# compbio-UofT/shrimp

Measured on AMD Instinct MI355X. Metric: reads/sec mapped (whole node), 100bp LS reads vs 3Gbp ref, 1/2/4/8 GPUs, higher is better.
Workload: dtype int16

## Files before the change

shrimp_amd/csrc/gm_lookup5.hip:

```cpp
#include <algorithm>
#include <cmath>
#include <mutex>
#include "gm_common.h"
#include "gm_internal.h"
#include <rocprim/device/device_scan.hpp>

typedef uint32_t k5_u32x4 __attribute__((ext_vector_type(4), aligned(4)));
typedef __attribute__((address_space(3))) uint32_t k5_lds_u32;
#define K5_LDS(off) ((k5_lds_u32*)(uintptr_t)(uint32_t)(off))
typedef __attribute__((address_space(3))) uint16_t k5_lds_u16;
#define K5_LDS16(off) ((k5_lds_u16*)(uintptr_t)(uint32_t)(off))
#define K5_LDS_OR(off, m) __hip_atomic_fetch_or(K5_LDS(off), (m), __ATOMIC_RELAXED, __HIP_MEMORY_SCOPE_WORKGROUP)

#ifndef K5_Q
#define K5_Q 4
#endif
enum { C_NCAND = 0, C_OVERFLOW, C_NMEMB, C_NKEEP, C_NSTRIP, C_NEDGE, C_NLISTS , C_SINK = 8, C_NRAW = 9, C_NDEFER = 10, C_NCAND0 = 11 , C_SPILL = 12 , C_WORDS = 16 };
#define K5_MAX_ROUNDS 4

#ifdef K5_STAMPS
__device__ unsigned long long k5_stamps[16];
#define K5_STAMP(i) do { if (tid == 0) { const unsigned long long t_ = __builtin_amdgcn_s_memtime(); atomicAdd(&k5_stamps[i], t_ - t_prev); t_prev = t_; } } while (0)
extern "C" int gm_debug_k5_stamps(unsigned long long* out) {
  unsigned long long z[16] = {0, 0, 0, 0, 0, 0, 0, 0, 0, 0, 0, 0, 0, 0, 0, 0};
  if (hipMemcpyFromSymbol(out, HIP_SYMBOL(k5_stamps), sizeof z) != hipSuccess) return GM_E_NODEVICE;
  if (hipMemcpyToSymbol(HIP_SYMBOL(k5_stamps), z, sizeof z) != hipSuccess) return GM_E_NODEVICE;
  return GM_OK;
}
#else
#define K5_STAMP(i) do { } while (0)
#endif

#ifdef GM_TUNING
__device__ unsigned long long k5_paths[3];
extern "C" int gm_debug_k5_paths(unsigned long long* out) {
  unsigned long long z[3] = {0, 0, 0};
  if (hipMemcpyFromSymbol(out, HIP_SYMBOL(k5_paths), sizeof z) != hipSuccess) return GM_E_NODEVICE;
  if (hipMemcpyToSymbol(HIP_SYMBOL(k5_paths), z, sizeof z) != hipSuccess) return GM_E_NODEVICE;
  return GM_OK;
}
#endif

struct K5Args {
  const uint32_t* reads; int n_reads, read_len, read_words, max_n_kmers, NL;
  int lsw, ltw;
  int cand_cap, hbits;
  int cand_limit;
  int xrec;
  int rounds; uint32_t round_regs;
  uint2* spill; int spill_cap;
  uint64_t* out; uint32_t* out_cnt; int out_cap; uint32_t* surv_cnt;
  int prune; uint32_t D; int e_max;
  uint32_t* heavy_list; uint32_t* heavy_cnt; int heavy_cap;
  unsigned long long* stats;
  uint32_t* fb_list; uint32_t* fb_cnt; int fb_cap;
  uint32_t* start_flags; uint32_t start_epoch;
  uint64_t* raw_out; int raw_cap; uint32_t* surv_seg; int n_slabs; uint32_t* pl_list; uint32_t* pl_cnt; int pl_cap;
};

__device__ __forceinline__ uint32_t k5_lane_times(int lane, uint32_t W) {
  uint32_t r; asm("v_mul_u32_u24 %0, %1, %2" : "=v"(r) : "v"(lane), "s"(W)); return r;
}

#include "gm_region_table.h"

#define K5_KERNEL_HEAD template <int LSWC> __global__ void __launch_bounds__(1024) k_lookup_v5(GmIndexDev ix, K5Args a)
#define K5_KERNEL_MULTI false
#include "gm_lookup5_kernel.inc"
#undef K5_KERNEL_HEAD
#undef K5_KERNEL_MULTI
#define K5_KERNEL_HEAD __global__ void __launch_bounds__(1024) __attribute__((amdgpu_waves_per_eu(5, 5))) k_lookup_v5_rounds(GmIndexDev ix, K5Args a)
#define K5_KERNEL_MULTI true
#define K5_KERNEL_LSWC 15
#include "gm_lookup5_kernel.inc"
#undef K5_KERNEL_HEAD
#undef K5_KERNEL_MULTI
#undef K5_KERNEL_LSWC
#define K5_KERNEL_HEAD __global__ void __launch_bounds__(1024) __attribute__((amdgpu_waves_per_eu(5, 5))) k_lookup_v5_half(GmIndexDev ix, K5Args a)
#define K5_KERNEL_MULTI true
#define K5_KERNEL_LSWC 14
#define K5_KERNEL_BLOOM true
#include "gm_lookup5_kernel.inc"
#undef K5_KERNEL_HEAD
#undef K5_KERNEL_BLOOM
#ifdef GM_TUNING
#define K5_KERNEL_HEAD __global__ void __launch_bounds__(1024) __attribute__((amdgpu_waves_per_eu(5, 5))) k_lookup_v5_half_plain(GmIndexDev ix, K5Args a)
#define K5_KERNEL_BLOOM false
#include "gm_lookup5_kernel.inc"
#undef K5_KERNEL_HEAD
#undef K5_KERNEL_BLOOM
#endif
#undef K5_KERNEL_MULTI
#undef K5_KERNEL_LSWC

__device__ __forceinline__ bool k5_strip(uint32_t p, int rb, uint32_t ovl) { return (p & ((1u << rb) - 1u)) < ovl && (p >> rb) > 0u; }

__global__ void __launch_bounds__(256) k_strip_count(const uint32_t* __restrict__ pos, uint32_t n_pos, int rb, uint32_t ovl, uint32_t* __restrict__ grp_cnt, uint32_t n_groups) {
  const uint32_t lane = threadIdx.x & 63u;
  uint64_t g = ((uint64_t)blockIdx.x * blockDim.x + threadIdx.x) >> 6;
  const uint64_t stride = ((uint64_t)gridDim.x * blockDim.x) >> 6;
  for (; g < n_groups; g += stride) {
    const uint64_t i = g * 64 + lane;
    const bool f = i < n_pos && k5_strip(pos[i], rb, ovl);
    const unsigned long long b = __ballot(f);
    if (lane == 0) grp_cnt[g] = (uint32_t)__popcll(b);
  }
}
__global__ void __launch_bounds__(256) k_strip_scatter(const uint32_t* __restrict__ pos, uint32_t n_pos, int rb, uint32_t ovl, const uint32_t* __restrict__ grp_rank,
                                                       uint32_t n_groups, uint32_t* __restrict__ spos) {
  const uint32_t lane = threadIdx.x & 63u;
  uint64_t g = ((uint64_t)blockIdx.x * blockDim.x + threadIdx.x) >> 6;
  const uint64_t stride = ((uint64_t)gridDim.x * blockDim.x) >> 6;
  for (; g < n_groups; g += stride) {
    const uint64_t i = g * 64 + lane;
    const uint32_t p = i < n_pos ? pos[i] : 0u;
    const bool f = i < n_pos && k5_strip(p, rb, ovl);
    const unsigned long long b = __ballot(f);
    if (f) spos[grp_rank[g] + (uint32_t)__popcll(b & ((1ull << lane) - 1ull))] = p;
  }
}
__global__ void __launch_bounds__(256) k_strip_dir(const uint32_t* __restrict__ dir, const uint32_t* __restrict__ pos, uint32_t n_pos, uint64_t K, int S, int rb, uint32_t ovl,
                                                   const uint32_t* __restrict__ grp_rank, uint32_t* __restrict__ sdir) {
  uint64_t k = (uint64_t)blockIdx.x * blockDim.x + threadIdx.x;
  const uint64_t stride = (uint64_t)gridDim.x * blockDim.x;
  for (; k <= K; k += stride) {
    const uint32_t i = dir[k * (uint64_t)S];
    uint32_t r = grp_rank[i >> 6];
    for (uint32_t q = i & ~63u; q < i; q++) r += k5_strip(pos[q], rb, ovl) ? 1u : 0u;
    sdir[k] = r;
  }
}

static std::mutex g_strip_mutex;
int gm_index_derive_strips(GmIndexHost* ix, hipStream_t stream) {
  std::lock_guard<std::mutex> lock(g_strip_mutex);
  if (ix->strips_ready) return GM_OK;
  const int rb = ix->params.region_bits; const uint32_t ovl = (uint32_t)ix->params.region_overlap;
  for (int sn = 0; sn < ix->n_seeds; sn++) {
    GmSeedHost& sd = ix->seeds[sn];
    const uint64_t K = 1ull << sd.kbits;
    const uint32_t n_groups = (uint32_t)(((uint64_t)sd.n_pos + 63) / 64) + 1u;
    uint32_t *d_cnt = nullptr, *d_rank = nullptr; void* tmp = nullptr; size_t tmp_bytes = 0;
    GM_HIP(hipMalloc(&d_cnt, (size_t)n_groups * 4)); GM_HIP(hipMalloc(&d_rank, (size_t)n_groups * 4));
    hipLaunchKernelGGL(k_strip_count, dim3(256 * 16), dim3(256), 0, stream, sd.d_pos, sd.n_pos, rb, ovl, d_cnt, n_groups);
    hipError_t e = rocprim::exclusive_scan(nullptr, tmp_bytes, d_cnt, d_rank, 0u, (size_t)n_groups, rocprim::plus<uint32_t>(), stream);
    if (e != hipSuccess) { gm_set_error("exclusive_scan size query: %s", hipGetErrorString(e)); return GM_E_NODEVICE; }
    GM_HIP(hipMalloc(&tmp, tmp_bytes ? tmp_bytes : 16));
    e = rocprim::exclusive_scan(tmp, tmp_bytes, d_cnt, d_rank, 0u, (size_t)n_groups, rocprim::plus<uint32_t>(), stream);
    if (e != hipSuccess) { gm_set_error("exclusive_scan: %s", hipGetErrorString(e)); return GM_E_NODEVICE; }
    uint32_t total = 0;
    GM_HIP(hipMemcpyAsync(&total, d_rank + (n_groups - 1), 4, hipMemcpyDeviceToHost, stream));
    GM_HIP(hipStreamSynchronize(stream));
    sd.n_spos = total;
    GM_HIP(hipMalloc(&sd.d_spos, ((size_t)total + 64) * 4));
    GM_HIP(hipMemsetAsync(sd.d_spos, 0xff, ((size_t)total + 64) * 4, stream));
    GM_HIP(hipMalloc(&sd.d_sdir, (size_t)(K + 1 + 16) * 4));
    hipLaunchKernelGGL(k_strip_scatter, dim3(256 * 16), dim3(256), 0, stream, sd.d_pos, sd.n_pos, rb, ovl, d_rank, n_groups, sd.d_spos);
    hipLaunchKernelGGL(k_strip_dir, dim3(256 * 16), dim3(256), 0, stream, sd.d_dir, sd.d_pos, sd.n_pos, K, ix->n_slabs, rb, ovl, d_rank, sd.d_sdir);
    GM_HIP(hipGetLastError());
    GM_HIP(hipStreamSynchronize(stream));
    (void)hipFree(d_cnt); (void)hipFree(d_rank); (void)hipFree(tmp);
  }
  ix->strips_ready = true;
  return GM_OK;
}

int gm_lookup5_launch(const GmIndexDev& ix, const uint32_t* d_reads, int n_reads, int read_len, int read_words, int max_n_kmers, int NL,
                      uint64_t* d_out, uint32_t* d_out_cnt, int out_cap, uint32_t* d_surv_cnt, int prune, uint32_t D, int e_max,
                      uint32_t* d_heavy_list, uint32_t* d_heavy_cnt, int heavy_cap, unsigned long long* d_stats, hipStream_t stream, GmK1Scratch* K,
                      uint64_t* d_raw, int raw_cap, uint32_t* d_surv_seg) {
  int dev = 0; if (hipGetDevice(&dev) != hipSuccess) return 0;
  if (!ix.seed[0].sdir || ix.region_bits < 9 || ix.region_bits > 16 || NL <= 0) return 0;
  const bool forced = gm_tune("GM_K1_V5") != nullptr;
  double entries = 0;
  for (int sn = 0; sn < ix.n_seeds; sn++) {
    const double lists = std::max(0, read_len - ix.seed[sn].span + 1 - ix.colour);
    entries += lists * (double)ix.seed[sn].n_pos / (double)(1ull << (ix.hflag ? 2 * GM_HASH_TABLE_POWER : 2 * ix.seed[sn].weight));
  }
  if (!forced && entries < 8000.0) return 0;
  const size_t budget = 160 * 1024 - 512;
  const size_t fixed0 = (size_t)24 * NL + 2 * (size_t)((read_len + 15) & ~15) + C_WORDS * 4 + GM_MAX_SEEDS * 32;
  const size_t full_tables = (size_t)(4u << 15) + (size_t)(4u << 12);
  int xrec = read_len > 128 ? 16 : 64;
  if (fixed0 + 24 * (size_t)xrec + full_tables > budget && fixed0 + 24 * 16 + full_tables <= budget) xrec = (int)((budget - full_tables - fixed0) / 24);
  const size_t fixed = fixed0 + 24 * (size_t)xrec;
  int lsw = 15;
  int threads = 1024;
  bool small_shape = false;
  if (!forced && ix.colour && NL <= 512 && !gm_tune("GM_K5_LSW") && !gm_tune("GM_K1_THREADS") && !(gm_tune("GM_K5_SMALL") && atoi(gm_tune("GM_K5_SMALL")) == 0)) {
    const double lam = entries * (double)((1u << ix.region_bits) + ix.region_overlap) / std::max(1.0, (double)ix.total_len);
    const double memb = 2.0 * entries * std::min(1.0, lam), late = 0.5 * entries * std::min(1.0, entries / (double)(32ull << 14));
    const double first = entries * std::min(1.0, (late + 0.5 * memb) / (double)(32ull << 11));
    const double cap14 = (double)(((4u << 14) / 4u / 6u) & ~15u);
    if (memb + late + first <= 0.5 * cap14 && fixed + (size_t)(4u << 14) + (size_t)(4u << 11) <= 96 * 1024) { small_shape = true; lsw = 14; threads = 512; }
  }
  int half = 0;
  if (const char* e = gm_tune("GM_K5_HALF")) half = atoi(e);
  const size_t half_budget = 80 * 1024 - 512, half_tables = (size_t)(4u << 14) + (size_t)(4u << 11);
  if (half && (ix.region_bits < 11 || NL > 512 || fixed0 + 24 * 8 + half_tables > half_budget)) half = 0;
  if (half) { lsw = 14; threads = 512; xrec = (int)std::min<size_t>(64, (half_budget - half_tables - fixed0) / 24); }
  if (half) if (const char* e = gm_tune("GM_K5_HALF_THREADS")) threads = std::max(64, std::min(1024, atoi(e) & ~63));
  const size_t fixed_h = fixed0 + 24 * (size_t)xrec;
  if (!half)
  if (const char* e = gm_tune("GM_K5_LSW")) lsw = std::max(8, std::min(15, atoi(e)));
  while (!half && lsw >= 8 && fixed + (size_t)(4u << lsw) + (size_t)(4u << (lsw - 3)) > budget) lsw--;
  if (lsw < 8) return 0;
  if (!half)
  if (const char* e = gm_tune("GM_K1_THREADS")) { const int v = std::max(64, std::min(1024, atoi(e))); threads = 64; while (threads * 2 <= v) threads *= 2; }
  const int ltw = lsw - 3;
  const int hbits = lsw - 2;
  const int cand_cap = (int)(((4u << lsw) / 4u / 6u) & ~15u);
  if (cand_cap < 16) return 0;
  int cand_limit = cand_cap - 8, rounds = 1;
  if (!forced) {
    const double lam = entries * (double)((1u << ix.region_bits) + ix.region_overlap) / std::max(1.0, (double)ix.total_len);
    const double memb = 2.0 * entries * std::min(1.0, lam), late = 0.5 * entries * std::min(1.0, entries / (double)(32ull << (lsw + (half == 1 ? 1 : 0))));
    const double first = entries * std::min(1.0, (late + 0.5 * memb) / (double)(32ull << (lsw - 3)));
    if (memb + late + first > 0.85 * cand_cap) {
      rounds = (int)std::ceil((memb + late + first) / ((half ? 0.95 : 1.25) * cand_cap));
      rounds = std::max(rounds, 2);
      if (rounds > K5_MAX_ROUNDS || NL > threads || lsw != (half ? 14 : 15)) return 0;
    }
  }
  if (const char* e = gm_tune("GM_K5_ROUNDS")) { rounds = std::max(1, std::min(K5_MAX_ROUNDS, atoi(e))); if (rounds > 1 && (NL > threads || lsw != (half ? 14 : 15))) return 0; }
  const uint32_t n_regs = (uint32_t)((ix.total_len + (1ull << ix.region_bits) - 1) >> ix.region_bits);
  const uint32_t round_regs = std::max(1u, (n_regs + (uint32_t)rounds - 1u) / (uint32_t)rounds);
  if (const char* e = gm_tune("GM_K5_CANDLIMIT")) cand_limit = std::max(1, std::min(cand_limit, atoi(e)));
  if (prune && (D + (uint32_t)std::max(0, e_max) > (1u << ix.region_bits) || D > 0xFFFFu)) return 0;
  const size_t lds = (half ? fixed_h : fixed) + (size_t)(4u << lsw) + (size_t)(4u << ltw);
  const int fb_cap = std::max(4096, 2 * n_reads);
  if (!K->cus) { if (hipDeviceGetAttribute(&K->cus, hipDeviceAttributeMultiprocessorCount, dev) != hipSuccess || K->cus < 1) K->cus = 256; }
  if (fb_cap > K->k5_cap) {
    if (K->k5_fb) { (void)hipStreamSynchronize(stream); (void)hipFree(K->k5_fb); (void)hipFree(K->k5_pl); K->k5_fb = nullptr; K->k5_pl = nullptr; K->k5_cap = 0; }
    if (hipMalloc(&K->k5_fb, (size_t)(fb_cap + 4) * 4) != hipSuccess) return 0;
    if (hipMalloc(&K->k5_pl, (size_t)(fb_cap + 4) * 4) != hipSuccess) return 0;
    K->k5_cap = fb_cap;
  }
  uint32_t* const fb_cnt_p = K->k5_fb + K->k5_cap; uint32_t* const pl_cnt_p = K->k5_pl + K->k5_cap;
  if (hipMemsetAsync(fb_cnt_p, 0, 4, stream) != hipSuccess || hipMemsetAsync(pl_cnt_p, 0, 4, stream) != hipSuccess) return GM_E_NODEVICE;
  if (gm_lds_at_least((const void*)k_lookup_v5<15>, lds) != hipSuccess || gm_lds_at_least((const void*)k_lookup_v5<14>, lds) != hipSuccess ||
      gm_lds_at_least((const void*)k_lookup_v5_rounds, lds) != hipSuccess || gm_lds_at_least((const void*)k_lookup_v5_half, lds) != hipSuccess ||
#ifdef GM_TUNING
      gm_lds_at_least((const void*)k_lookup_v5_half_plain, lds) != hipSuccess ||
#endif
      gm_lds_at_least((const void*)k_lookup_v5<0>, lds) != hipSuccess) return 0;
  int grid = std::min(2 * n_reads, (half || small_shape) ? 2 * K->cus : K->cus);
  if (const char* e = gm_tune("GM_K5_GRID")) grid = std::max(1, std::min(2 * n_reads, atoi(e)));
  K5Args a;
  a.reads = d_reads; a.n_reads = n_reads; a.read_len = read_len; a.read_words = read_words; a.max_n_kmers = max_n_kmers; a.NL = NL;
  a.lsw = lsw; a.ltw = ltw; a.cand_cap = cand_cap; a.hbits = hbits; a.cand_limit = cand_limit; a.xrec = xrec; a.rounds = rounds; a.round_regs = round_regs;
  a.out = d_out; a.out_cnt = d_out_cnt; a.out_cap = out_cap; a.surv_cnt = d_surv_cnt; a.prune = prune; a.D = D; a.e_max = e_max;
  a.heavy_list = d_heavy_list; a.heavy_cnt = d_heavy_cnt; a.heavy_cap = heavy_cap; a.stats = d_stats;
  a.fb_list = K->k5_fb; a.fb_cnt = fb_cnt_p; a.fb_cap = fb_cap;
  a.raw_out = prune ? d_raw : nullptr; a.raw_cap = raw_cap; a.surv_seg = d_surv_seg; a.n_slabs = ix.n_slabs; a.pl_list = K->k5_pl; a.pl_cnt = pl_cnt_p; a.pl_cap = fb_cap;
  a.spill = nullptr; a.spill_cap = cand_cap;
  if (rounds > 1) {
    const size_t need = (size_t)grid * (size_t)(rounds - 1) * (size_t)cand_cap;
    if (need > K->k5_spill_n) {
      if (K->k5_spill) { (void)hipStreamSynchronize(stream); (void)hipFree(K->k5_spill); K->k5_spill = nullptr; K->k5_spill_n = 0; }
      if (hipMalloc(&K->k5_spill, need * sizeof(uint2)) != hipSuccess) return 0;
      K->k5_spill_n = need;
    }
    a.spill = K->k5_spill;
  }
  const bool use_flags = K->start_flags && grid <= K->flag_cap;
  K->flag_grid = use_flags ? grid : 0;
  a.start_flags = use_flags ? K->start_flags : nullptr; a.start_epoch = K->epoch;
  K->rounds = rounds; K->half = half;
  if (half) {
#ifdef GM_TUNING
    if (half == 2) hipLaunchKernelGGL(k_lookup_v5_half_plain, dim3(grid), dim3(threads), lds, stream, ix, a); else
#endif
    hipLaunchKernelGGL(k_lookup_v5_half, dim3(grid), dim3(threads), lds, stream, ix, a);
  } else if (rounds > 1) hipLaunchKernelGGL(k_lookup_v5_rounds, dim3(grid), dim3(threads), lds, stream, ix, a);
  else if (lsw == 15) hipLaunchKernelGGL((k_lookup_v5<15>), dim3(grid), dim3(threads), lds, stream, ix, a);
  else if (lsw == 14) hipLaunchKernelGGL((k_lookup_v5<14>), dim3(grid), dim3(threads), lds, stream, ix, a);
  else hipLaunchKernelGGL((k_lookup_v5<0>), dim3(grid), dim3(threads), lds, stream, ix, a);
  if (hipGetLastError() != hipSuccess) return GM_E_NODEVICE;
  return 1;
}
```

shrimp_amd/csrc/gm_lookup5_kernel.inc:

```
K5_KERNEL_HEAD {
  constexpr bool MULTI = K5_KERNEL_MULTI;
#ifdef K5_KERNEL_BLOOM
  constexpr bool BLOOM = K5_KERNEL_BLOOM;
#else
  constexpr bool BLOOM = false;
#endif
#ifdef K5_KERNEL_LSWC
  constexpr int LSWC = K5_KERNEL_LSWC;
#endif
  if (a.start_flags && threadIdx.x == 0) __hip_atomic_store(&a.start_flags[blockIdx.x], a.start_epoch, __ATOMIC_RELAXED, __HIP_MEMORY_SCOPE_SYSTEM);
  __builtin_amdgcn_s_setprio(3);
  extern __shared__ __align__(16) uint32_t smem[];
  const int tid = threadIdx.x, nthr = blockDim.x, lane = tid & (GM_WAVE - 1);
  const int wv = __builtin_amdgcn_readfirstlane(tid >> 6), nwv = nthr >> 6;
  const int S = ix.n_slabs, rb = ix.region_bits, lsw = LSWC ? LSWC : a.lsw, ltw = lsw - 3, hbits = lsw - 2;
  const int cand_cap = LSWC ? (int)(((4u << LSWC) / 4u / 6u) & ~15u) : a.cand_cap;
  const uint32_t rmask = (1u << rb) - 1u, ovl = (uint32_t)ix.region_overlap;
  const uint32_t wmask = (1u << lsw) - 1u, tmask = (1u << ltw) - 1u;
  if ((uint32_t)(uintptr_t)(k5_lds_u32*)smem != 0u) __builtin_trap();
  uint32_t* twice = smem;
  uint32_t* seen = smem + (1u << ltw);
  uint32_t* candp = seen;
  uint16_t* candy = (uint16_t*)(candp + cand_cap);
  uint32_t* htag = seen + (1u << hbits);
  uint32_t* hmin = htag + (1u << hbits);
  uint32_t* hmax = hmin + (1u << hbits);
  uint32_t* rec = seen + (1u << lsw);
  const int RC = a.NL + a.xrec;
  uint32_t* srec = rec + 4 * RC;
  uint8_t* codes = (uint8_t*)(srec + 2 * RC);
  uint32_t* ctrl = (uint32_t*)(codes + 2 * ((a.read_len + 15) & ~15));
  const uint32_t smask4 = wmask << 2, tmask4 = tmask << 2, swb = 4u << ltw;
  const int sh_a = rb - 2, sh_b = rb + lsw;
  const uint32_t hmask = (1u << hbits) - 1u; const int hshift = 32 - hbits;
  const uint32_t pb_cap = MULTI ? (2u << hbits) : (uint32_t)cand_cap;
  const uint32_t pb_pos = MULTI ? swb + (4u << hbits) : swb, pb_y = pb_pos + 4u * pb_cap;
  uint32_t* const sb_pos = MULTI ? htag : candp; uint16_t* const sb_y = (uint16_t*)(sb_pos + pb_cap);
  const int hclr_q = (int)(3u << hbits) >> 2;
  const int tab_q = (int)(((1u << ltw) + (1u << lsw)) >> 2);
  const uint32_t* __restrict__ pos0 = ix.seed[0].pos;
  const uint32_t* __restrict__ spos0 = ix.seed[0].spos;
  unsigned long long my_lookups = 0, my_entries = 0;
  uint32_t k_prune = __builtin_amdgcn_readfirstlane(a.prune != 0 ? 1u : 0u), k_D = __builtin_amdgcn_readfirstlane(a.D);
  uint32_t k_emax_on = __builtin_amdgcn_readfirstlane(a.e_max >= 0 ? 1u : 0u), k_emax = __builtin_amdgcn_readfirstlane((uint32_t)max(a.e_max, 0));
  asm volatile("" : "+s"(k_prune), "+s"(k_D), "+s"(k_emax_on), "+s"(k_emax));

  { uint4* t4 = (uint4*)smem; for (int w = tid; w < tab_q; w += nthr) t4[w] = make_uint4(0, 0, 0, 0); }
  if (tid < C_WORDS) ctrl[tid] = 0;

  auto bloom_mask = [&](const uint32_t t) -> uint32_t { return (1u << (t & 31u)) | (2u << ((t + (((t >> 5) & 3u) << 2)) & 31u)); };
  auto mark = [&](const uint32_t p) {
    const uint32_t av = p >> sh_a, t = p >> sh_b, m1 = 1u << (t & 31u), m = BLOOM ? bloom_mask(t) : m1;
    const uint32_t old = K5_LDS_OR(swb + (av & smask4), m);
    if ((old & m) == m) K5_LDS_OR(av & tmask4, m1);
  };
  auto has2 = [&](const uint32_t p) -> bool { return (*K5_LDS((p >> sh_a) & tmask4) >> ((p >> sh_b) & 31u)) & 1u; };
  auto has2r = [&](const uint32_t r) -> bool {
#ifdef K5_NO_TWICE_FILTER
    return true;
#else
    return (*K5_LDS((r << 2) & tmask4) >> ((r >> lsw) & 31u)) & 1u;
#endif
  };

#ifdef K5_STAMPS
  unsigned long long t_prev = __builtin_amdgcn_s_memtime();
#endif
  const bool ahead = a.NL <= nthr;
  const uint32_t cpad = (uint32_t)((a.read_len + 15) & ~15);
  uint32_t pf_b = 0, pf_e = 0, pf_sb = 0, pf_se = 0; bool pf_ok = false;
  auto fill_codes = [&](const int r, uint8_t* cb) {
    if (r >= 2 * a.n_reads) return;
    const uint32_t* rw = a.reads + (size_t)(r >> 1) * a.read_words;
    for (int i = tid; i < a.read_len; i += nthr) cb[i] = (uint8_t)gm_read_code(rw, a.read_len, (r & 1) ^ ix.cs_flip, ix.colour, i, GM_READ_RNA(ix, r >> 1));
  };
  uint32_t* stab = ctrl + C_WORDS;
  if (tid < ix.n_seeds) {
    const GmSeedDev& sd = ix.seed[tid];
    const uint64_t d = (uint64_t)(uintptr_t)sd.dir, sdp = (uint64_t)(uintptr_t)sd.sdir, po = (uint64_t)(sd.pos - pos0), so = (uint64_t)(sd.spos - spos0);
    *(uint4*)&stab[8 * tid] = make_uint4((uint32_t)d, (uint32_t)(d >> 32), (uint32_t)sdp, (uint32_t)(sdp >> 32));
    *(uint4*)&stab[8 * tid + 4] = make_uint4((uint32_t)po, (uint32_t)(po >> 32), (uint32_t)so, (uint32_t)(so >> 32));
  }
  int k_sn = 0, k_i = 0, k_span = 0; uint64_t k_mask = 0; bool k_ok = false;
  const int k_stride = 1, k_slot = tid;
  const int nsw = ahead ? min(nwv, (a.NL + GM_WAVE - 1) / GM_WAVE) : nwv;
  if (ahead && k_slot < a.NL) {
    k_sn = k_slot / a.max_n_kmers; k_i = k_slot - k_sn * a.max_n_kmers;
    k_span = ix.seed[k_sn].span; k_mask = ix.seed[k_sn].mask;
    k_ok = k_i >= ix.colour && k_i + k_span <= a.read_len;
    if (!k_ok) { k_span = 0; k_mask = 0; }
  }
  uint32_t* cnl_w = nullptr;
  auto strip_of = [&](const int j0, uint32_t& slen) -> const uint32_t* {
    const uint2 sr = *(const uint2*)&srec[2 * j0];
    const uint4 st = *(const uint4*)&stab[8 * (rec[4 * j0 + 3] & 15u) + 4];
    slen = sr.y;
    return spos0 + ((((uint64_t)st.w << 32) | st.z) + sr.x);
  };
  auto put_records = [&](const uint64_t la, const uint32_t len, const uint32_t ysn, const uint32_t sb, const uint32_t slen) {
    const uint32_t nch = (len + 255u) >> 8;
    const uint32_t j = atomicAdd(cnl_w, nch);
    for (uint32_t c = 0; c < nch && j + c < (uint32_t)RC; c++) {
      const uint64_t ca = la + ((uint64_t)c << 10);
      *(uint4*)&rec[4 * (j + c)] = make_uint4((uint32_t)ca, (uint32_t)(ca >> 32), min(256u, len - (c << 8)), ((ysn >> 12) & 0xFFF0u) | (ysn & 0xFu));
      *(uint2*)&srec[2 * (j + c)] = c ? make_uint2(0u, 0u) : make_uint2(sb, slen);
    }
  };
  auto put_list = [&](const uint32_t b, const uint32_t n, const uint32_t sb, const uint32_t sn) {
    const uint4 so = *(const uint4*)&stab[8 * k_sn + 4];
    const uint64_t ptr = (((uint64_t)so.y << 32) | so.x) + b;
    put_records((uint64_t)(uintptr_t)(pos0 + ptr), n, ((uint32_t)k_i << 16) | (uint32_t)k_sn, sb, sn);
  };
  auto kmer_ahead = [&](const int r, const uint8_t* cb) {
    pf_ok = k_ok && r < 2 * a.n_reads;
    uint32_t mapidx = 0;
    if (wv >= nsw) {}
    else if (!ix.hflag) {
      for (int t0 = 0; t0 < ix.max_seed_span; t0 += 8) {
        uint32_t c[8];
#pragma unroll
        for (int u = 0; u < 8; u++) { const int x = k_i + k_span - 1 - t0 - u; c[u] = cb[min(max(x, 0), a.read_len - 1)]; }
#pragma unroll
        for (int u = 0; u < 8; u++) mapidx = ((k_mask >> (t0 + u)) & 1ull) ? ((mapidx << 2) | (c[u] & 3u)) : mapidx;
      }
    } else if (pf_ok) mapidx = gm_mapidx(ix, k_mask, k_span, cb + k_i);
    if (!pf_ok) mapidx = 0;
    const uint4 sp = *(const uint4*)&stab[8 * k_sn];
    typedef const uint32_t __attribute__((address_space(1)))* k5_gptr;
    const k5_gptr dir = (k5_gptr)(((uint64_t)sp.y << 32) | sp.x) + (size_t)mapidx * (uint32_t)S;
    const k5_gptr sdir = (k5_gptr)(((uint64_t)sp.w << 32) | sp.z) + mapidx;
    pf_b = dir[0]; pf_e = dir[S]; pf_sb = sdir[0]; pf_se = sdir[1];
  };
  uint32_t rf_lo[K5_MAX_ROUNDS], rf_m1[K5_MAX_ROUNDS];
#pragma unroll
  for (int d = 0; d < K5_MAX_ROUNDS; d++) {
    const uint64_t rsz64 = 1ull << rb, lo = (uint64_t)d * a.round_regs * rsz64, hi = d >= a.rounds - 1 ? (1ull << 32) : lo + (uint64_t)a.round_regs * rsz64;
    const uint64_t flo = lo >= rsz64 ? lo - rsz64 : 0ull, fhi = hi + rsz64 < (1ull << 32) ? hi + rsz64 : (1ull << 32);
    rf_lo[d] = (uint32_t)std::min<uint64_t>(flo, 0xFFFFFFFFull); rf_m1[d] = MULTI && d < a.rounds && flo < (1ull << 32) ? (uint32_t)(fhi - 1ull - flo) : 0u;
  }
  uint2* const spill_wg = MULTI ? a.spill + (size_t)blockIdx.x * (size_t)(a.rounds - 1) * a.spill_cap : nullptr;
  __syncthreads();
  if (ahead) { fill_codes(blockIdx.x, codes); __syncthreads(); kmer_ahead(blockIdx.x, codes); }
  int it = 0;
  for (int rs = blockIdx.x; rs < 2 * a.n_reads; rs += gridDim.x, it++) {
    uint32_t* const cnl = &ctrl[C_NLISTS + (it & 1)];
    cnl_w = cnl;
    if (ahead) {
      fill_codes(rs + (int)gridDim.x, codes + (uint32_t)((it + 1) & 1) * cpad);
      const uint32_t b = pf_b, e = pf_e, sb = pf_sb, se = pf_se;
      if ((b ^ e ^ sb ^ se) == 0x9E3779B9u && e - b == 0x7F4A7C15u) ctrl[C_SINK] = 1u;
      const bool has_list = pf_ok && e != b && e - b <= ix.list_cutoff;
      if (pf_ok) my_lookups++;
      if (has_list) { my_entries += (e - b); put_list(b, e - b, sb, se - sb); }
      __syncthreads();
      K5_STAMP(8);
      kmer_ahead(rs + (int)gridDim.x, codes + (uint32_t)((it + 1) & 1) * cpad);
      K5_STAMP(9);
    } else {
    const int rd = rs >> 1, st = rs & 1;
    const uint32_t* rw = a.reads + (size_t)rd * a.read_words;
    for (int i = tid; i < a.read_len; i += nthr) codes[i] = (uint8_t)gm_read_code(rw, a.read_len, st ^ ix.cs_flip, ix.colour, i, GM_READ_RNA(ix, rd));
    __syncthreads();
    for (int off = tid; off < a.NL; off += nthr) {
      const int sn = off / a.max_n_kmers, i = off - sn * a.max_n_kmers;
      const int span = ix.seed[sn].span;
      if (i < ix.colour || i + span > a.read_len) continue;
      const uint32_t mapidx = gm_mapidx(ix, ix.seed[sn].mask, span, codes + i);
      const uint32_t* dir = ix.seed[sn].dir + (size_t)mapidx * (uint32_t)S;
      my_lookups++;
      const uint32_t b = dir[0], e = dir[S];
      if (e == b || e - b > ix.list_cutoff) continue;
      const uint32_t sb = ix.seed[sn].sdir[mapidx], se = ix.seed[sn].sdir[mapidx + 1];
      my_entries += (e - b);
      put_records((uint64_t)(uintptr_t)(ix.seed[sn].pos + b), e - b, ((uint32_t)i << 16) | (uint32_t)sn, sb, se - sb);
    }
    __syncthreads();
    }
    K5_STAMP(0);
    const int nl_raw = (int)*cnl, nl = min(nl_raw, RC);
    const bool rec_over = nl_raw > RC;

    struct Step { uint32_t n, ysn; const uint32_t* src; };
// ... 99 lines not shown
            const uint32_t o2 = K5_LDS_OR(swb + (a2 & smask4), m2);
            if (W > 3) o3 = K5_LDS_OR(swb + (a3 & smask4), m3);
            if (BLOOM) {
              K5_TWICE(a0, (o0 & m0) == m0 ? b0 : 0u);
              K5_TWICE(a1, (o1 & m1) == m1 ? b1 : 0u);
              K5_TWICE(a2, (o2 & m2) == m2 ? b2 : 0u);
              if (W > 3) K5_TWICE(a3, (o3 & m3) == m3 ? b3 : 0u);
            } else {
            K5_TWICE(a0, o0 & m0);
            K5_TWICE(a1, o1 & m1);
            K5_TWICE(a2, o2 & m2);
            if (W > 3) K5_TWICE(a3, o3 & m3);
            }
#endif
          }
          gen(sd[q]); issue(sd[q], sv[q]);
        }
      }
#ifdef K5_ABL_A_TWICE
      if (a_rep == 0) { __syncthreads(); K5_STAMP(12); }
#endif
    }
    Step sdB[K5_Q]; k5_u32x4 svB[K5_Q];
    K5_GEN_RESET_B();
#pragma unroll
    for (int q = 0; q < K5_Q; q++) { K5_GEN_B(sdB[q]); issue(sdB[q], svB[q]); }
    __syncthreads();
    K5_STAMP(1);
    bool fallback = false;
    uint32_t nc = 0;
    const int nrounds = MULTI ? a.rounds : 1;
      {
      if (!MULTI) { uint4* h4 = (uint4*)htag; for (int w = tid; w < hclr_q; w += nthr) h4[w] = make_uint4(0, 0, 0, 0); }
      {
        for (int j0 = tid >> 2; j0 <
#ifdef K5_ABL_NOSTRIP
             0
#else
             nl
#endif
             ; j0 += nthr >> 2) {
          uint32_t slen; const uint32_t* sp = strip_of(j0, slen);
          const uint32_t ysn = rec[4 * j0 + 3];
          for (uint32_t e = (uint32_t)(tid & 3) * 4u; e < slen; e += 16u) {
            const k5_u32x4 v = *(const k5_u32x4*)(sp + e);
            const uint32_t nv = min(4u, slen - e);
            const bool a0 = !has2(v.x) && has2(v.x - (1u << rb));
            const bool a1 = nv > 1 && !has2(v.y) && has2(v.y - (1u << rb));
            const bool a2 = nv > 2 && !has2(v.z) && has2(v.z - (1u << rb));
            const bool a3 = nv > 3 && !has2(v.w) && has2(v.w - (1u << rb));
            const bool c0 = a0, c1 = a1, c2 = a2, c3 = a3;
            if (c0 | c1 | c2 | c3) {
              uint32_t idx = atomicAdd(&ctrl[C_NCAND], (uint32_t)c0 + (uint32_t)c1 + (uint32_t)c2 + (uint32_t)c3);
              if (idx + 4u <= pb_cap) {
                const uint16_t y16 = (uint16_t)ysn;
                if (c0) { sb_pos[idx] = v.x; sb_y[idx++] = y16; }
                if (c1) { sb_pos[idx] = v.y; sb_y[idx++] = y16; }
                if (c2) { sb_pos[idx] = v.z; sb_y[idx++] = y16; }
                if (c3) { sb_pos[idx] = v.w; sb_y[idx++] = y16; }
              }
            }
          }
        }
        Step (&sd)[K5_Q] = sdB; k5_u32x4 (&sv)[K5_Q] = svB;
        while (sd[0].n) {
  #pragma unroll
          for (int q = 0; q < K5_Q; q++) {
            const Step& s = sd[q];
            K5_WAIT_OLDEST(sv[q]);
            const uint32_t W = (s.n + 63u) >> 6;
            const uint32_t e0 = k5_lane_times(lane, W);
            const uint32_t mine = min(W, __builtin_elementwise_sub_sat(s.n, e0));
  #ifdef K5_ABL_B
            const uint32_t t0 = 0, t1 = 0, t2 = 0, b3 = ((sv[q].x ^ sv[q].y ^ sv[q].z ^ sv[q].w) == 0x12345678u) << 3;
  #else
            const uint32_t t0 = *K5_LDS((sv[q].x >> sh_a) & tmask4), t1 = *K5_LDS((sv[q].y >> sh_a) & tmask4);
            const uint32_t t2 = *K5_LDS((sv[q].z >> sh_a) & tmask4);
            uint32_t b3 = 0;
            if (W > 3u) b3 = __builtin_amdgcn_ubfe(*K5_LDS((sv[q].w >> sh_a) & tmask4), __builtin_amdgcn_ubfe(sv[q].w, sh_b, 5), 1) << 3;
  #endif
            uint32_t hits = (__builtin_amdgcn_ubfe(t0, __builtin_amdgcn_ubfe(sv[q].x, sh_b, 5), 1) | (__builtin_amdgcn_ubfe(t1, __builtin_amdgcn_ubfe(sv[q].y, sh_b, 5), 1) << 1) |
                             (__builtin_amdgcn_ubfe(t2, __builtin_amdgcn_ubfe(sv[q].z, sh_b, 5), 1) << 2) | b3) &
                            ((1u << mine) - 1u);
            const uint32_t cnt = (uint32_t)__popc(hits);
            if (cnt) {
              const uint32_t ci = atomicAdd(&ctrl[C_NCAND], cnt);
              if (ci + cnt <= pb_cap) {
                uint32_t y16 = s.ysn;
                asm volatile("" : "+v"(y16));
                const uint32_t c1 = ci + (hits & 1u), c2 = ci + (uint32_t)__popc(hits & 3u), c3 = ci + (uint32_t)__popc(hits & 7u);
                if (hits & 1u) { *K5_LDS(pb_pos + (ci << 2)) = sv[q].x; *K5_LDS16(pb_y + (ci << 1)) = (uint16_t)y16; }
                if (hits & 2u) { *K5_LDS(pb_pos + (c1 << 2)) = sv[q].y; *K5_LDS16(pb_y + (c1 << 1)) = (uint16_t)y16; }
                if (hits & 4u) { *K5_LDS(pb_pos + (c2 << 2)) = sv[q].z; *K5_LDS16(pb_y + (c2 << 1)) = (uint16_t)y16; }
                if (hits & 8u) { *K5_LDS(pb_pos + (c3 << 2)) = sv[q].w; *K5_LDS16(pb_y + (c3 << 1)) = (uint16_t)y16; }
              }
            }
            K5_GEN_B(sd[q]); issue(sd[q], sv[q]);
          }
        }
        asm volatile("s_waitcnt vmcnt(0)" ::: "memory");
      }
      }
      __syncthreads();
      if (MULTI) {
        const uint32_t na_raw = ctrl[C_NCAND];
        if (na_raw + 8u > pb_cap) fallback = true;
        const uint32_t na = min(na_raw, pb_cap);
        const unsigned long long below = (1ull << lane) - 1ull;
        for (uint32_t i0 = 0; i0 < na; i0 += nthr) {
          const uint32_t i = i0 + tid;
          const bool live = i < na;
          const uint32_t p = *K5_LDS(pb_pos + ((live ? i : 0u) << 2)), ys = *K5_LDS16(pb_y + ((live ? i : 0u) << 1));
#pragma unroll
          for (int d = 0; d < K5_MAX_ROUNDS; d++) if (d < nrounds) {
            const bool in = live && p - rf_lo[d] <= rf_m1[d];
            const unsigned long long bi = __ballot(in);
            if (bi) {
              uint32_t base = 0;
              if (lane == 0) base = atomicAdd(&ctrl[d == 0 ? C_NCAND0 : C_SPILL + d - 1], (uint32_t)__popcll(bi));
              base = __builtin_amdgcn_readfirstlane(base);
              const uint32_t j = base + (uint32_t)__popcll(bi & below);
              if (in) {
                if (d == 0) { if (j < (uint32_t)cand_cap) { candp[j] = p; candy[j] = (uint16_t)ys; } }
                else if (j < (uint32_t)a.spill_cap) spill_wg[(size_t)(d - 1) * a.spill_cap + j] = make_uint2(p, ys);
              }
            }
          }
        }
        __syncthreads();
        { uint4* h4 = (uint4*)htag; for (int w = tid; w < hclr_q; w += nthr) h4[w] = make_uint4(0, 0, 0, 0); }
        __syncthreads();
      }
    for (int rd = 0; rd < nrounds; rd++) {
      uint32_t c_lo = 0, c_m1 = 0xFFFFFFFFu, f_lo = 0, f_m1 = 0xFFFFFFFFu;
      if (MULTI) {
        const uint64_t rsz64 = 1ull << rb, lo = (uint64_t)rd * a.round_regs * rsz64, hi = rd == nrounds - 1 ? (1ull << 32) : lo + (uint64_t)a.round_regs * rsz64;
        const uint64_t flo = lo >= rsz64 ? lo - rsz64 : 0ull, fhi = hi + rsz64 < (1ull << 32) ? hi + rsz64 : (1ull << 32);
        c_lo = (uint32_t)lo; c_m1 = (uint32_t)(hi - 1ull - lo); f_lo = (uint32_t)flo; f_m1 = (uint32_t)(fhi - 1ull - flo);
      }
      auto in_core = [&](const uint32_t p) -> bool { return !MULTI || p - c_lo <= c_m1; };
      if (MULTI && rd > 0) {
        const uint32_t ns_raw = ctrl[C_SPILL + rd - 1];
        if (ns_raw > (uint32_t)a.spill_cap || ns_raw > (uint32_t)a.cand_limit) fallback = true;
        const uint32_t nsp = min(ns_raw, (uint32_t)min(a.spill_cap, cand_cap));
        const unsigned long long* src = (const unsigned long long*)(spill_wg + (size_t)(rd - 1) * a.spill_cap);
        for (uint32_t i0 = 0; i0 < nsp; i0 += 6u * (uint32_t)nthr) {
          unsigned long long v[6];
#pragma unroll
          for (int k = 0; k < 6; k++) { const uint32_t i = i0 + (uint32_t)k * (uint32_t)nthr + (uint32_t)tid; v[k] = __hip_atomic_load(src + min(i, nsp - 1u), __ATOMIC_RELAXED, __HIP_MEMORY_SCOPE_AGENT); }
#pragma unroll
          for (int k = 0; k < 6; k++) { const uint32_t i = i0 + (uint32_t)k * (uint32_t)nthr + (uint32_t)tid; if (i < nsp) { candp[i] = (uint32_t)v[k]; candy[i] = (uint16_t)(v[k] >> 32); } }
        }
        { uint4* h4 = (uint4*)htag; for (int w = tid; w < hclr_q; w += nthr) h4[w] = make_uint4(0, 0, 0, 0); }
        if (tid == 0) { ctrl[C_NCAND] = ns_raw; ctrl[C_NSTRIP] = 0; ctrl[C_NEDGE] = 0; ctrl[C_NDEFER] = 0; }
      }
      if (rd > 0) __syncthreads();
      K5_STAMP(2);
      const uint32_t nc_raw = ctrl[(MULTI && rd == 0) ? C_NCAND0 : C_NCAND];
      if (nc_raw > (uint32_t)a.cand_limit) fallback = true;
      nc = min(nc_raw, (uint32_t)cand_cap);
      uint32_t* const elist = rec; const uint32_t ecap = 6u * (uint32_t)RC;
      uint32_t* const dlist = elist + (uint32_t)RC; const uint32_t scap = (uint32_t)RC, dcap = ecap - scap;
      auto settle = [&](const uint32_t i, const uint32_t h, const uint32_t off) {
        atomicMax(&hmin[h], 0x10000u - off); atomicMax(&hmax[h], off + 1u);
        candp[i] = (h << 16) | off;
      };
      auto probe_on = [&](const uint32_t i) {
        const uint32_t p = candp[i], r = p >> rb, off = p & rmask;
        const uint32_t h = k5_insert(htag, hmask, hshift, r, true, true);
        if (h != 0xFFFFFFFFu) {
          settle(i, h, off);
          if (off < ovl && r > 0 && k5_insert(htag, hmask, hshift, r - 1u, false) == 0xFFFFFFFFu) ctrl[C_OVERFLOW] = 1u;
        } else ctrl[C_OVERFLOW] = 1u;
      };
      if (!fallback) {
        for (uint32_t i0 = 0; i0 < nc; i0 += nthr) {
          const uint32_t i = i0 + tid;
          const bool live = i < nc;
          const uint32_t p = candp[live ? i : 0u], r = p >> rb, off = p & rmask, r1 = r + 1u;
          const uint32_t h0 = k5_hash(r1, hshift);
          uint32_t prev = 0xFFFFFFFFu;
          if (live) prev = atomicCAS(&htag[h0], 0u, (r1 << 8) | K5_FA | K5_FC);
          const bool hit = live && (prev == 0u || (prev >> 8) == r1);
          if (hit) {
            if (prev != 0u) k5_again(htag, h0, prev, true);
            settle(i, h0, off);
          }
          const bool strip = hit && off < ovl && r > 0, later = live && !hit;
          const unsigned long long bs = __ballot(strip), bd = __ballot(later);
          if (bs | bd) {
            uint32_t sb = 0, db = 0;
            if (lane == 0) { if (bs) sb = atomicAdd(&ctrl[C_NSTRIP], (uint32_t)__popcll(bs)); if (bd) db = atomicAdd(&ctrl[C_NDEFER], (uint32_t)__popcll(bd)); }
            sb = __builtin_amdgcn_readfirstlane(sb); db = __builtin_amdgcn_readfirstlane(db);
            const unsigned long long below = (1ull << lane) - 1ull;
            if (strip) { const uint32_t j = sb + (uint32_t)__popcll(bs & below); if (j < scap) elist[j] = r - 1u; else ctrl[C_OVERFLOW] = 1u; }
            if (later) { const uint32_t j = db + (uint32_t)__popcll(bd & below); if (j < dcap) dlist[j] = i; else probe_on(i); }
          }
        }
      }
      __syncthreads();
      K5_STAMP(10);
      if (!fallback) {
        const uint32_t ns = min(ctrl[C_NSTRIP], scap), nd = min(ctrl[C_NDEFER], dcap);
#ifdef K5_1B_TWO_LOOPS
        for (uint32_t j = tid; j < nd; j += nthr) probe_on(dlist[j]);
        for (uint32_t j = tid; j < ns; j += nthr)
          if (k5_insert(htag, hmask, hshift, elist[j], false) == 0xFFFFFFFFu) ctrl[C_OVERFLOW] = 1u;
#else
        for (uint32_t j = tid; j < nd + ns; j += nthr) {
          const bool own = j < nd;
          const uint32_t v = *(own ? dlist + j : elist + (j - nd));
          const uint32_t p = candp[own ? v : 0u], r = own ? p >> rb : v, off = p & rmask;
          const uint32_t h = k5_insert(htag, hmask, hshift, r, own, own);
          if (h == 0xFFFFFFFFu) ctrl[C_OVERFLOW] = 1u;
          else if (own) {
            settle(v, h, off);
            if (off < ovl && r > 0 && k5_insert(htag, hmask, hshift, r - 1u, false) == 0xFFFFFFFFu) ctrl[C_OVERFLOW] = 1u;
          }
        }
#endif
      }
      __syncthreads();
      K5_STAMP(3);
      fallback = fallback || rec_over || ctrl[C_OVERFLOW] != 0u;
      if (!fallback) {
        unsigned long long* out = (unsigned long long*)a.out + (size_t)rs * a.out_cap;
        const uint32_t edge = a.D + (uint32_t)max(a.e_max, 0);
        auto emit = [&](const bool memb, const bool keep, const uint32_t p, const uint32_t i) {
          const unsigned long long bm = __ballot(memb), bk = __ballot(keep);
          if (bm) {
            uint32_t base = 0;
            if (lane == 0) { atomicAdd(&ctrl[C_NMEMB], (uint32_t)__popcll(bm)); if (bk) base = atomicAdd(&ctrl[C_NKEEP], (uint32_t)__popcll(bk)); }
            base = __builtin_amdgcn_readfirstlane(base);
            if (keep) {
              const uint32_t slot = base + (uint32_t)__popcll(bk & ((1ull << lane) - 1ull));
              const uint32_t y16 = candy[i];
              if (slot < (uint32_t)a.out_cap) out[slot] = ((unsigned long long)p << 32) | ((unsigned long long)(y16 >> 4) << 16) | (y16 & 15u);
            }
          }
        };
  #ifndef K5_2A_BRANCHY
        {
          const uint32_t do_prune = k_prune, Dv = k_D, emax_on = k_emax_on, emax = k_emax;
          const uint32_t rsz = 1u << rb;
          for (uint32_t i0 = 0; i0 < nc; i0 += nthr) {
            const uint32_t i = i0 + tid;
            const uint32_t valid = i < nc ? 1u : 0u;
            const uint32_t w = candp[valid ? i : 0u], h = w >> 16, off = w & 0xFFFFu;
            const uint32_t town = htag[h], mn = hmin[h], mx = hmax[h];
            const uint32_t r = (town >> 8) - 1u, p = (r << rb) | off;
            const uint32_t is_m = (town >> 1) & 1u , r_pos = r > 0u ? 1u : 0u;
            const uint32_t nb_m = do_prune & (((off < edge ? 1u : 0u) & r_pos) | (off + edge >= rsz ? 1u : 0u)), nb_o = (off < ovl ? 1u : 0u) & r_pos;
            const uint32_t core = in_core(p) ? 1u : 0u;
            const uint32_t nbv = valid & core & (is_m ? nb_m : nb_o);
            const bool nb = nbv != 0u;
            const unsigned long long bn = __ballot(nb);
            if (bn) {
              uint32_t base = 0;
              if (lane == 0) base = atomicAdd(&ctrl[C_NEDGE], (uint32_t)__popcll(bn));
              base = __builtin_amdgcn_readfirstlane(base);
              if (nb) {
                const uint32_t j = base + (uint32_t)__popcll(bn & ((1ull << lane) - 1ull));
                if (j < ecap) elist[j] = i; else ctrl[C_OVERFLOW] = 1u;
              }
            }
            const uint32_t fe = (town >> 4) & 1u , fd = (town >> 3) & 1u ;
            const uint32_t span = (mx - 1u) - (0x10000u - mn);
            const uint32_t iso = fe | (fd & (span <= Dv ? 1u : 0u));
            const uint32_t tight = emax_on & (span <= emax ? 1u : 0u);
            const uint32_t membv = valid & core & is_m & (nbv ^ 1u), keepv = membv & ((iso & (tight ^ 1u)) | (do_prune ^ 1u));
            emit(membv != 0u, keepv != 0u, p, i);
          }
        }
  #else
        for (uint32_t i0 = 0; i0 < nc; i0 += nthr) {
          const uint32_t i = i0 + tid;
          bool memb = false, keep = false; uint32_t p = 0;
          if (i < nc) {
            const uint32_t w = candp[i], h = w >> 16, off = w & 0xFFFFu, town = htag[h], r = (town >> 8) - 1u;
            p = (r << rb) | off;
            const bool is_m = (town & K5_FB) != 0u;
            const bool nb = is_m ? (a.prune && ((off < edge && r > 0) || off + edge >= (1u << rb))) : (off < ovl && r > 0);
            if (nb) {
              const uint32_t j = atomicAdd(&ctrl[C_NEDGE], 1u);
              if (j < ecap) elist[j] = i; else ctrl[C_OVERFLOW] = 1u;
            } else if (is_m) {
              memb = true; keep = true;
              if (a.prune) {
                const uint32_t co = (town & K5_FE) ? 3u : ((town & K5_FD) ? 2u : 1u);
                const uint32_t span = (hmax[h] - 1u) - (0x10000u - hmin[h]);
                keep = co >= 3u || (co == 2u && span <= a.D);
                if (keep && a.e_max >= 0 && span <= (uint32_t)a.e_max) keep = false;
              }
            }
          }
          emit(memb, keep, p, i);
        }
  #endif
        __syncthreads();
        K5_STAMP(11);
        const uint32_t ne = min(ctrl[C_NEDGE], ecap);
        for (uint32_t j0 = 0; j0 < ne; j0 += nthr) {
          const uint32_t j = j0 + tid;
          bool memb = false, keep = false; uint32_t p = 0, i = 0;
          if (j < ne) {
            i = elist[j];
            const uint32_t w = candp[i], hown = w >> 16, off = w & 0xFFFFu, town = htag[hown], r = (town >> 8) - 1u;
            p = (r << rb) | off;
            uint32_t tlf = 0, trt = 0;
            memb = (town & K5_FB) != 0u;
            uint32_t hlf = 0xFFFFFFFFu; bool have_lf = false;
            if (!memb && off < ovl && r > 0) { hlf = k5_find_maybe(htag, hmask, hshift, r - 1u, has2r(r - 1u), tlf); have_lf = true; memb = (tlf & K5_FB) != 0u; }
            if (memb) {
              keep = true;
              if (a.prune) {
                uint32_t hrt = 0xFFFFFFFFu; trt = 0;
                if (off < edge) { if (!have_lf && r > 0) hlf = k5_find_maybe(htag, hmask, hshift, r - 1u, has2r(r - 1u) | has2r(r - 2u), tlf); } else tlf = 0;
                if (off + edge >= (1u << rb)) hrt = k5_find(htag, hmask, hshift, r + 1u, trt);
                const uint32_t co = (town & K5_FE) ? 3u : ((town & K5_FD) ? 2u : 1u);
                const uint32_t omin = 0x10000u - hmin[hown], omax = hmax[hown] - 1u;
                const bool cl = (tlf & K5_FC) != 0u, cr = (trt & K5_FC) != 0u;
                const uint32_t rbase = r << rb;
                keep = co >= 3u || (co == 2u && omax - omin <= a.D);
                uint32_t lmin = 0, lmax = 0, rmin = 0, rmax = 0;
                if (cl) { lmin = 0x10000u - hmin[hlf]; lmax = hmax[hlf] - 1u; }
                if (cr) { rmin = 0x10000u - hmin[hrt]; rmax = hmax[hrt] - 1u; }
                if (!keep && cl) keep = p - (rbase - (1u << rb) + lmax) <= a.D;
                if (!keep && cr) keep = (rbase + (1u << rb) + rmin) - p <= a.D;
                if (keep && a.e_max >= 0) {
                  uint32_t gmin = rbase + omin, gmax = rbase + omax;
                  if (cl) gmin = rbase - (1u << rb) + lmin;
                  if (cr) gmax = rbase + (1u << rb) + rmax;
                  if (gmax - gmin <= (uint32_t)a.e_max) keep = false;
                }
              }
            }
          }
          emit(memb, keep, p, i);
        }
      }
      if (MULTI && rd + 1 < nrounds) { __syncthreads(); if (ctrl[C_OVERFLOW] != 0u) fallback = true; }
    }
    __syncthreads();
    if (ctrl[C_OVERFLOW] != 0u) fallback = true;
    bool prune_only = false;
    if (!fallback && a.prune && ctrl[C_NKEEP] > (uint32_t)a.out_cap) {
      if (!(MULTI && nrounds > 1) && a.raw_out && ctrl[C_NMEMB] <= (uint32_t)a.raw_cap) {
        prune_only = true;
        unsigned long long* raw = (unsigned long long*)a.raw_out + (size_t)rs * a.raw_cap;
        for (int sl = 0; sl < a.n_slabs; sl++) {
        for (uint32_t i0 = 0; i0 < nc; i0 += nthr) {
          const uint32_t i = i0 + tid;
          bool memb = false; uint32_t p = 0;
          if (i < nc) {
            const uint32_t w = candp[i], h = w >> 16, off = w & 0xFFFFu, town = htag[h], r = (town >> 8) - 1u;
            p = (r << rb) | off;
            if ((int)(p >> ix.slab_bits) == sl || (sl == a.n_slabs - 1 && (int)(p >> ix.slab_bits) >= a.n_slabs)) {
              memb = (town & K5_FB) != 0u;
              if (!memb && off < ovl && r > 0) { uint32_t tlf; k5_find_maybe(htag, hmask, hshift, r - 1u, has2r(r - 1u), tlf); memb = (tlf & K5_FB) != 0u; }
            }
          }
          const unsigned long long bm = __ballot(memb);
          if (bm) {
            uint32_t base = 0;
            if (lane == 0) base = atomicAdd(&ctrl[C_NRAW], (uint32_t)__popcll(bm));
            base = __builtin_amdgcn_readfirstlane(base);
            if (memb) {
              const uint32_t slot = base + (uint32_t)__popcll(bm & ((1ull << lane) - 1ull)), y16 = candy[i];
              if (slot < (uint32_t)a.raw_cap) raw[slot] = ((unsigned long long)p << 32) | ((unsigned long long)(y16 >> 4) << 16) | (y16 & 15u);
            }
          }
        }
        __syncthreads();
        if (tid == 0 && a.surv_seg) { if (sl == 0) a.surv_seg[(size_t)rs * (a.n_slabs + 1)] = 0u; a.surv_seg[(size_t)rs * (a.n_slabs + 1) + sl + 1] = ctrl[C_NRAW]; }
        }
      } else fallback = true;
    }
    K5_STAMP(4);
#ifdef K5_STAMPS
    if (tid == 0) { atomicAdd(&k5_stamps[6], (unsigned long long)nc); if (fallback) atomicAdd(&k5_stamps[7], 1ull); }
#endif
#ifdef GM_TUNING
    if (tid == 0 && (fallback || prune_only)) atomicAdd(&k5_paths[fallback ? 1 : 2], 1ull);
#endif
    if (tid == 0) {
      if (fallback) {
        const uint32_t f = atomicAdd(a.fb_cnt, 1u);
        if (f < (uint32_t)a.fb_cap) a.fb_list[f] = (uint32_t)rs; else GS_ADD(a.stats, GS_OVERFLOW_SURV, 1ull);
      } else if (prune_only) {
        const uint32_t nm = ctrl[C_NRAW];
        a.surv_cnt[rs] = nm;
        GS_ADD(a.stats, GS_SURVIVORS, (unsigned long long)nm);
        const uint32_t f = atomicAdd(a.pl_cnt, 1u);
        if (f < (uint32_t)a.pl_cap) a.pl_list[f] = (uint32_t)rs; else GS_ADD(a.stats, GS_OVERFLOW_SURV, 1ull);
      } else {
        const uint32_t nm = ctrl[C_NMEMB], nk = ctrl[C_NKEEP];
        a.surv_cnt[rs] = nm;
        GS_ADD(a.stats, GS_SURVIVORS, (unsigned long long)nm);
        if (a.prune) GS_ADD(a.stats, GS_PRUNED, (unsigned long long)(nm - nk));
        const bool heavy = nk > (uint32_t)a.out_cap;
        if (a.prune) a.out_cnt[rs] = heavy ? 0xFFFFFFFFu : nk;
        if (heavy) {
          const uint32_t hs = atomicAdd(a.heavy_cnt, 1u);
          if (hs < (uint32_t)a.heavy_cap) a.heavy_list[hs] = (uint32_t)rs; else GS_ADD(a.stats, GS_OVERFLOW_SURV, 1ull);
        }
      }
      for (int c = 0; c < C_NLISTS; c++) ctrl[c] = 0;
      *cnl = 0; ctrl[C_NRAW] = 0; ctrl[C_NDEFER] = 0; if (MULTI) ctrl[C_NCAND0] = 0;
      if (MULTI) for (int d = 0; d < K5_MAX_ROUNDS - 1; d++) ctrl[C_SPILL + d] = 0;
    }
    { uint4* t4 = (uint4*)smem; for (int w = tid; w < tab_q; w += nthr) t4[w] = make_uint4(0, 0, 0, 0); }
    K5_STAMP(5);
  }
#ifdef GM_TUNING
  if (tid == 0 && it > 0) atomicAdd(&k5_paths[0], (unsigned long long)it);
#endif
  for (int d = GM_WAVE / 2; d > 0; d >>= 1) { my_lookups += __shfl_down(my_lookups, d); my_entries += __shfl_down(my_entries, d); }
  if (lane == 0) { GS_ADD(a.stats, GS_LOOKUPS, my_lookups); GS_ADD(a.stats, GS_ENTRIES, my_entries); }
}
```

Measured before the change: 3.507 million.

## Replace block-wide strip/defer lists with per-wave LDS lists, dropping a block barrier

Deferred-probe and strip entries no longer go into block-shared lists indexed through LDS atomic counters. Each wave now appends them to its own slice of the record buffer using ballot/popcount offsets and drains that slice itself. This removes the global atomics and one __syncthreads between the first pass and the insert pass, so each wave does its own deferred work. In exchange, per-wave capacity is smaller, so a skewed wave may overflow its slice and fall back to inline probing or insertion. Load balance across waves may also get worse.

```diff
diff --git a/shrimp_amd/csrc/gm_lookup5.hip b/shrimp_amd/csrc/gm_lookup5.hip
--- a/shrimp_amd/csrc/gm_lookup5.hip
+++ b/shrimp_amd/csrc/gm_lookup5.hip
@@ -15,7 +15,7 @@
 #ifndef K5_Q
 #define K5_Q 4
 #endif
-enum { C_NCAND = 0, C_OVERFLOW, C_NMEMB, C_NKEEP, C_NSTRIP, C_NEDGE, C_NLISTS , C_SINK = 8, C_NRAW = 9, C_NDEFER = 10, C_NCAND0 = 11 , C_SPILL = 12 , C_WORDS = 16 };
+enum { C_NCAND = 0, C_OVERFLOW, C_NMEMB, C_NKEEP, C_WLISTED , C_NEDGE, C_NLISTS , C_SINK = 8, C_NRAW = 9, C_WSPOT = 10 , C_NCAND0 = 11 , C_SPILL = 12 , C_WORDS = 16 };
 #define K5_MAX_ROUNDS 4
 
 #ifdef K5_STAMPS
@@ -39,6 +39,13 @@
   if (hipMemcpyToSymbol(HIP_SYMBOL(k5_paths), z, sizeof z) != hipSuccess) return GM_E_NODEVICE;
   return GM_OK;
 }
+__device__ unsigned long long k5_wave_lists[2];
+extern "C" int gm_debug_k5_wave_lists(unsigned long long* out) {
+  unsigned long long z[2] = {0, 0};
+  if (hipMemcpyFromSymbol(out, HIP_SYMBOL(k5_wave_lists), sizeof z) != hipSuccess) return GM_E_NODEVICE;
+  if (hipMemcpyToSymbol(HIP_SYMBOL(k5_wave_lists), z, sizeof z) != hipSuccess) return GM_E_NODEVICE;
+  return GM_OK;
+}
 #endif
 
 struct K5Args {
@@ -47,6 +54,7 @@
   int cand_cap, hbits;
   int cand_limit;
   int xrec;
+  int wlist;
   int rounds; uint32_t round_regs;
   uint2* spill; int spill_cap;
   uint64_t* out; uint32_t* out_cnt; int out_cap; uint32_t* surv_cnt;
@@ -254,6 +262,8 @@
   a.fb_list = K->k5_fb; a.fb_cnt = fb_cnt_p; a.fb_cap = fb_cap;
   a.raw_out = prune ? d_raw : nullptr; a.raw_cap = raw_cap; a.surv_seg = d_surv_seg; a.n_slabs = ix.n_slabs; a.pl_list = K->k5_pl; a.pl_cnt = pl_cnt_p; a.pl_cap = fb_cap;
   a.spill = nullptr; a.spill_cap = cand_cap;
+  a.wlist = 0x7FFFFFFF;
+  if (const char* e = gm_tune("GM_K5_WLIST")) a.wlist = std::max(0, atoi(e));
   if (rounds > 1) {
     const size_t need = (size_t)grid * (size_t)(rounds - 1) * (size_t)cand_cap;
     if (need > K->k5_spill_n) {
diff --git a/shrimp_amd/csrc/gm_lookup5_kernel.inc b/shrimp_amd/csrc/gm_lookup5_kernel.inc
--- a/shrimp_amd/csrc/gm_lookup5_kernel.inc
+++ b/shrimp_amd/csrc/gm_lookup5_kernel.inc
@@ -28,6 +28,15 @@
   uint32_t* rec = seen + (1u << lsw);
   const int RC = a.NL + a.xrec;
   uint32_t* srec = rec + 4 * RC;
+  const uint32_t wseg = 6u * (uint32_t)RC / (uint32_t)nwv;
+  uint32_t* const wlist = rec + (uint32_t)wv * wseg;
+#ifdef GM_TUNING
+  const uint32_t wcap = min(wseg, (uint32_t)__builtin_amdgcn_readfirstlane(a.wlist));
+#define K5_WL_COUNT(listed, spot) do { if (lane == 0) { atomicAdd(&ctrl[C_WLISTED], (listed)); atomicAdd(&ctrl[C_WSPOT], (spot)); } } while (0)
+#else
+  const uint32_t wcap = wseg;
+#define K5_WL_COUNT(listed, spot) do { } while (0)
+#endif
   uint8_t* codes = (uint8_t*)(srec + 2 * RC);
   uint32_t* ctrl = (uint32_t*)(codes + 2 * ((a.read_len + 15) & ~15));
   const uint32_t smask4 = wmask << 2, tmask4 = tmask << 2, swb = 4u << ltw;
@@ -433,7 +442,7 @@
           for (int k = 0; k < 6; k++) { const uint32_t i = i0 + (uint32_t)k * (uint32_t)nthr + (uint32_t)tid; if (i < nsp) { candp[i] = (uint32_t)v[k]; candy[i] = (uint16_t)(v[k] >> 32); } }
         }
         { uint4* h4 = (uint4*)htag; for (int w = tid; w < hclr_q; w += nthr) h4[w] = make_uint4(0, 0, 0, 0); }
-        if (tid == 0) { ctrl[C_NCAND] = ns_raw; ctrl[C_NSTRIP] = 0; ctrl[C_NEDGE] = 0; ctrl[C_NDEFER] = 0; }
+        if (tid == 0) { ctrl[C_NCAND] = ns_raw; ctrl[C_NEDGE] = 0; }
       }
       if (rd > 0) __syncthreads();
       K5_STAMP(2);
@@ -441,7 +450,6 @@
       if (nc_raw > (uint32_t)a.cand_limit) fallback = true;
       nc = min(nc_raw, (uint32_t)cand_cap);
       uint32_t* const elist = rec; const uint32_t ecap = 6u * (uint32_t)RC;
-      uint32_t* const dlist = elist + (uint32_t)RC; const uint32_t scap = (uint32_t)RC, dcap = ecap - scap;
       auto settle = [&](const uint32_t i, const uint32_t h, const uint32_t off) {
         atomicMax(&hmin[h], 0x10000u - off); atomicMax(&hmax[h], off + 1u);
         candp[i] = (h << 16) | off;
@@ -455,6 +463,7 @@
         } else ctrl[C_OVERFLOW] = 1u;
       };
       if (!fallback) {
+        uint32_t wn = 0;
         for (uint32_t i0 = 0; i0 < nc; i0 += nthr) {
           const uint32_t i = i0 + tid;
           const bool live = i < nc;
@@ -468,29 +477,25 @@
             settle(i, h0, off);
           }
           const bool strip = hit && off < ovl && r > 0, later = live && !hit;
-          const unsigned long long bs = __ballot(strip), bd = __ballot(later);
-          if (bs | bd) {
-            uint32_t sb = 0, db = 0;
-            if (lane == 0) { if (bs) sb = atomicAdd(&ctrl[C_NSTRIP], (uint32_t)__popcll(bs)); if (bd) db = atomicAdd(&ctrl[C_NDEFER], (uint32_t)__popcll(bd)); }
-            sb = __builtin_amdgcn_readfirstlane(sb); db = __builtin_amdgcn_readfirstlane(db);
-            const unsigned long long below = (1ull << lane) - 1ull;
-            if (strip) { const uint32_t j = sb + (uint32_t)__popcll(bs & below); if (j < scap) elist[j] = r - 1u; else ctrl[C_OVERFLOW] = 1u; }
-            if (later) { const uint32_t j = db + (uint32_t)__popcll(bd & below); if (j < dcap) dlist[j] = i; else probe_on(i); }
-          }
-        }
-      }
-      __syncthreads();
-      K5_STAMP(10);
-      if (!fallback) {
-        const uint32_t ns = min(ctrl[C_NSTRIP], scap), nd = min(ctrl[C_NDEFER], dcap);
-#ifdef K5_1B_TWO_LOOPS
-        for (uint32_t j = tid; j < nd; j += nthr) probe_on(dlist[j]);
-        for (uint32_t j = tid; j < ns; j += nthr)
-          if (k5_insert(htag, hmask, hshift, elist[j], false) == 0xFFFFFFFFu) ctrl[C_OVERFLOW] = 1u;
-#else
-        for (uint32_t j = tid; j < nd + ns; j += nthr) {
-          const bool own = j < nd;
-          const uint32_t v = *(own ? dlist + j : elist + (j - nd));
+          const unsigned long long bi = __ballot(strip | later);
+          if (bi) {
+            const uint32_t j = wn + (uint32_t)__popcll(bi & ((1ull << lane) - 1ull));
+            wn += (uint32_t)__popcll(bi);
+            if (strip | later) {
+              if (j < wcap) wlist[j] = later ? i : (0x80000000u | (r - 1u));
+              else if (later) probe_on(i);
+              else if (k5_insert(htag, hmask, hshift, r - 1u, false) == 0xFFFFFFFFu) ctrl[C_OVERFLOW] = 1u;
+            }
+          }
+        }
+        K5_STAMP(10);
+        __builtin_amdgcn_wave_barrier();
+        const uint32_t nw = min(wn, wcap);
+        K5_WL_COUNT(nw, wn - nw);
+        for (uint32_t j = lane; j < nw; j += GM_WAVE) {
+          const uint32_t w = wlist[j];
+          const bool own = (w >> 31) == 0u;
+          const uint32_t v = w & 0x7FFFFFFFu;
           const uint32_t p = candp[own ? v : 0u], r = own ? p >> rb : v, off = p & rmask;
           const uint32_t h = k5_insert(htag, hmask, hshift, r, own, own);
           if (h == 0xFFFFFFFFu) ctrl[C_OVERFLOW] = 1u;
@@ -499,7 +504,6 @@
             if (off < ovl && r > 0 && k5_insert(htag, hmask, hshift, r - 1u, false) == 0xFFFFFFFFu) ctrl[C_OVERFLOW] = 1u;
           }
         }
-#endif
       }
       __syncthreads();
       K5_STAMP(3);
@@ -663,6 +667,7 @@
 #endif
 #ifdef GM_TUNING
     if (tid == 0 && (fallback || prune_only)) atomicAdd(&k5_paths[fallback ? 1 : 2], 1ull);
+    if (tid == 0) { atomicAdd(&k5_wave_lists[0], (unsigned long long)ctrl[C_WLISTED]); atomicAdd(&k5_wave_lists[1], (unsigned long long)ctrl[C_WSPOT]); ctrl[C_WSPOT] = 0; }
 #endif
     if (tid == 0) {
       if (fallback) {
@@ -687,7 +692,7 @@
         }
       }
       for (int c = 0; c < C_NLISTS; c++) ctrl[c] = 0;
-      *cnl = 0; ctrl[C_NRAW] = 0; ctrl[C_NDEFER] = 0; if (MULTI) ctrl[C_NCAND0] = 0;
+      *cnl = 0; ctrl[C_NRAW] = 0; if (MULTI) ctrl[C_NCAND0] = 0;
       if (MULTI) for (int d = 0; d < K5_MAX_ROUNDS - 1; d++) ctrl[C_SPILL + d] = 0;
     }
     { uint4* t4 = (uint4*)smem; for (int w = tid; w < tab_q; w += nthr) t4[w] = make_uint4(0, 0, 0, 0); }
@@ -699,3 +704,4 @@
   for (int d = GM_WAVE / 2; d > 0; d >>= 1) { my_lookups += __shfl_down(my_lookups, d); my_entries += __shfl_down(my_entries, d); }
   if (lane == 0) { GS_ADD(a.stats, GS_LOOKUPS, my_lookups); GS_ADD(a.stats, GS_ENTRIES, my_entries); }
 }
+#undef K5_WL_COUNT
```

After: 3.573 million, median of 6. 1.9% higher.
